# wukailu/single-stable-dreamfusion

Hardware: AMD Instinct MI355X
Metric: SDS train steps/sec + rays/sec at 128×128, 1/2/4/8 MI355X (higher is better)
Workload: dtype fp16+f32; 1 GPU; C2: -O (fp16, cuda_ray, dir_text) 128x128 render, batch 1, max_steps 512, density grid update every 16 steps; global_batch=1, parallelism=dp1, backward=fused, launch=hip-graph replay, grad_exchange=none (one rank), optimizer_in_graph=True

## Files before the change

### include/dfhip.h

```cpp
#ifndef DFHIP_H
#define DFHIP_H

#include <stdint.h>

#ifdef __cplusplus
extern "C" {
#endif

typedef void *dfhip_stream_t;

enum dfhip_dtype { DFHIP_F32 = 0, DFHIP_F16 = 1, DFHIP_F64 = 2, DFHIP_BF16 = 3 };
enum dfhip_shading {
    DFHIP_SHADING_ALBEDO = 0,
    DFHIP_SHADING_TEXTURELESS = 1,
    DFHIP_SHADING_LAMBERTIAN = 2,
    DFHIP_SHADING_NORMAL = 3
};

enum dfhip_status {
    DFHIP_OK = 0,
    DFHIP_EINVAL = 1,
    DFHIP_EDTYPE = 2,
    DFHIP_ELAUNCH = 3,
    DFHIP_ENOMEM = 4
// ... 444 lines not shown
                                              const int32_t *m_dev, uint32_t D, uint32_t C,
                                              uint32_t L, float S, uint32_t H, uint32_t gridtype,
                                              int align_corners, uint32_t group, float eps,
                                              uint32_t *entries, uint32_t *counts,
                                              float *partial, int accumulate,
                                              dfhip_stream_t stream);
typedef struct dfhip_binned_opts {
    int32_t walk_mode;
    int32_t fast_bin;
    int32_t walk_groups_per_cu;
    int32_t lane_perm;
    int32_t kept_clean;
    uint64_t *trace;
    float *found_inf;
    const uint32_t *row_live;
} dfhip_binned_opts;
int dfhip_grid_backward_binned_scratch_opts(uint32_t cap, const int32_t *offsets_host,
                                            uint32_t L, uint32_t C, uint32_t group,
                                            const dfhip_binned_opts *opts, uint64_t *entries_u32,
                                            uint64_t *counts_u32, uint64_t *partial_f32);
uint32_t dfhip_grid_backward_binned_tile(uint32_t group, const dfhip_binned_opts *opts);
int dfhip_grid_encode_backward_binned_opts(int phase, int grad_dtype, const void *grad_lbc,
                                           const float *inputs, float bound,
                                           const int32_t *offsets, const int32_t *offsets_host,
                                           float *grad_embeddings, uint32_t B,
                                           const int32_t *m_dev, uint32_t D, uint32_t C,
                                           uint32_t L, float S, uint32_t H, uint32_t gridtype,
                                           int align_corners, uint32_t group, float eps,
                                           uint32_t *entries, uint32_t *counts, float *partial,
                                           int accumulate, const dfhip_binned_opts *opts,
// ... 68 lines not shown
    const float *nears, const float *fars, const float *w1, const float *b1, const float *w2,
    const float *b2, float *out_image, float *out_depth, uint8_t *mask, const float *g_image,
    float *grad_image, float *grad_ws, float *partial, float *gw1, float *gb1, float *gw2,
    float *gb2, const float *grad_loss, float lambda, float *loss, float *found_inf,
    int defer_sum, dfhip_stream_t stream);

int dfhip_ray_chain_train(
    int rgb_dtype, const float *sigmas, const void *rgbs, const float *deltas,
    const int32_t *rays, uint32_t M, uint32_t N, float T_thresh, float *ws, float *depth,
    float *image, const float *rays_d, const float *nears, const float *fars, const float *w1,
    const float *b1, const float *w2, const float *b2, float *out_image, float *out_depth,
    uint8_t *mask, const float *g_image, float *grad_image, float *grad_ws, float *partial,
    float *gw1, float *gb1, float *gw2, float *gb2, const float *grad_loss, float lambda,
    float *loss, float *found_inf, int defer_sum, float *grad_sigmas, void *grad_rgbs,
    dfhip_stream_t stream);

int dfhip_entropy_forward(uint32_t N, const float *ws, float lambda, float *loss,
                          dfhip_stream_t stream);
int dfhip_entropy_backward(uint32_t N, const float *ws, const float *grad_loss, float lambda,
                           float *grad_ws, dfhip_stream_t stream);
int dfhip_entropy_backward_accumulate(uint32_t N, const float *ws, const float *grad_loss,
                                      float lambda, float *grad_ws, dfhip_stream_t stream);
int dfhip_opacity_forward(uint32_t N, const float *ws, float lambda, float *loss, int accumulate,
                          dfhip_stream_t stream);
int dfhip_opacity_backward_accumulate(uint32_t N, const float *ws, const float *grad_loss,
                                      float lambda, float *grad_ws, dfhip_stream_t stream);

int dfhip_train_step_prologue(const float *pose, float fx, float fy, float cx, float cy,
                              uint32_t H, uint32_t W, const float *aabb, float min_near,
                              uint64_t seed, uint64_t step, int perturb, const float *alphas,
// ... 141 lines not shown
```

### single-stable-dreamfusion_amd/_dfhip.py

```python
from __future__ import annotations

import ctypes
import os
from pathlib import Path

import torch

LIB_PATH = Path(os.environ.get("DFHIP_LIB", Path(__file__).resolve().parent / "lib" / "libdfhip.so"))

F32, F16, F64, BF16 = 0, 1, 2, 3
_DTYPE = {torch.float32: F32, torch.float16: F16, torch.float64: F64, torch.bfloat16: BF16}

_vp, _u32, _i32, _f32 = ctypes.c_void_p, ctypes.c_uint32, ctypes.c_int, ctypes.c_float
_u64 = ctypes.c_uint64

_SIGS = {
    "dfhip_near_far_from_aabb": [_i32, _vp, _vp, _vp, _u32, _f32, _vp, _vp, _vp],
    "dfhip_get_rays": [_vp, _f32, _f32, _f32, _f32, _u32, _u32, _vp, _vp, _vp],
    "dfhip_density_grid_ema": [_vp, _vp, _u32, _u32, _f32, _vp, _vp, _vp],
    "dfhip_packbits_mean": [_vp, _u32, _vp, _f32, _vp, _vp, _vp],
    "dfhip_mean_count": [_vp, _u32, _vp, _vp],
    "dfhip_sph_from_ray": [_i32, _vp, _vp, _f32, _u32, _vp, _vp],
    "dfhip_morton3D": [_vp, _u32, _vp, _vp],
    "dfhip_morton3D_invert": [_vp, _u32, _vp, _vp],
# ... 127 lines not shown
        _vp, _vp, _f32, _vp, _vp, _vp, _vp, _vp, _vp, _vp, _vp, _i32, _u32, _vp, _vp, _vp, _u32,
        _vp, _vp, _vp, _vp, _vp, _vp, _vp, _u32, _u32, _f32, _u32, _u32, _i32, _vp, _vp, _u32,
        _vp],
    "dfhip_adam_amp_step": [_i32, _vp, _vp, _vp, _vp, _vp, _vp, _vp, _vp, _vp, _vp, _vp, _vp,
                            _vp, _vp, _f32, _f32, _i32, _vp],
    "dfhip_adam_amp_step_lr_dev": [_i32, _vp, _vp, _vp, _vp, _vp, _vp, _vp, _vp, _vp, _vp, _vp,
                                   _vp, _vp, _vp, _vp, _f32, _f32, _i32, _vp],
    "dfhip_adam_amp_step_tail": [_i32, _vp, _vp, _vp, _vp, _vp, _vp, _vp, _vp, _vp, _vp, _vp,
                                 _vp, _vp, _vp, _vp, _f32, _f32, _i32, _u32, _vp, _vp, _vp, _vp],
    "dfhip_ray_head_backward_check": [_u32, _vp, _vp, _vp, _vp, _vp, _vp, _vp, _vp, _vp, _vp,
                                      _vp, _vp, _vp, _vp, _vp, _vp, _vp, _f32, _vp, _vp, _vp],
    "dfhip_ray_head_forward_backward_entropy_loss_check": [_u32] + [_vp] * 22 + [_f32, _vp, _vp,
                                                                                 _i32, _vp],
    "dfhip_ray_chain_train": [_i32] + [_vp] * 4 + [_u32, _u32, _f32] + [_vp] * 22 + [
        _f32, _vp, _vp, _i32, _vp, _vp, _vp],
    "dfhip_param_grad_sums": [_vp, _u32, _vp, _vp, _vp, _vp, _vp, _vp, _i32, _u32, _vp, _vp, _vp,
                              _vp, _vp, _vp, _f32, _vp, _vp, _vp],
    "dfhip_grid_field_backward_check": [_i32, _vp, _vp, _f32, _vp, _vp, _vp, _vp, _vp, _vp, _vp,
                                        _vp, _i32, _u32, _vp, _vp, _vp, _u32, _vp, _vp, _vp, _vp,
                                        _vp, _vp, _i32, _vp, _i32, _vp],
    "dfhip_grid_field_backward_check_live": [_i32, _vp, _vp, _f32, _vp, _vp, _vp, _vp, _vp, _vp,
                                             _vp, _vp, _i32, _u32, _vp, _vp, _vp, _u32, _vp, _vp,
                                             _vp, _vp, _vp, _vp, _i32, _vp, _i32, _vp, _vp],
    "dfhip_march_rays_train_count_staged_quads": [_i32, _vp, _vp, _vp, _f32, _f32, _u32, _u32,
                                                  _u32, _u32, _vp, _vp, _vp, _vp, _vp, _vp, _vp,
                                                  _i32, _vp, _vp, _u32, _f32, _u32, _u32, _i32,
                                                  _u32, _vp, _vp, _vp],
    "dfhip_train_step_prologue_row": [_vp, _f32, _f32, _f32, _f32, _u32, _u32, _vp, _f32,
                                      ctypes.c_uint64, ctypes.c_uint64, _i32, _vp, _u32, _u32,
                                      _vp, _vp, _vp, _vp, _vp, _vp, _vp, _vp, _vp, _u32, _vp,
# ... 249 lines not shown
```

### single-stable-dreamfusion_amd/_gridencoder.py

```python
import ctypes

import _dfhip as _d
from _dfhip import call, ptr, stream, checked


def _common(inputs, embeddings, offsets):
    checked(inputs, "inputs")
    if inputs.dtype.itemsize != 4 or not inputs.is_floating_point():
        raise RuntimeError("inputs must be a float32 tensor")
    checked(embeddings, "embeddings")
    checked(offsets, "offsets", "int")
    return _d.dtype_code(embeddings, "embeddings")


def grid_encode_forward(inputs, embeddings, offsets, outputs, B, D, C, L, S, H, dy_dx, gridtype,
                        align_corners):
    dt = _common(inputs, embeddings, offsets)
    checked(outputs, "outputs")
    call("dfhip_grid_encode_forward", dt, ptr(inputs), ptr(embeddings), ptr(offsets), ptr(outputs),
         B, D, C, L, S, H, ptr(dy_dx), gridtype, int(bool(align_corners)), stream())


def grid_encode_backward(grad, inputs, embeddings, offsets, grad_embeddings, B, D, C, L, S, H,
                         dy_dx, grad_inputs, gridtype, align_corners):
# ... 90 lines not shown
    checked(partial, "partial")
    if m_dev is not None:
        checked(m_dev, "m_dev", "int")
    call("dfhip_grid_encode_backward_sliced_dyn", _d.dtype_code(grad_lbc, "grad"),
         _d.dtype_code(grad_embeddings, "grad_embeddings"), ptr(grad_lbc), ptr(inputs),
         float(bound), ptr(offsets), ptr(grad_embeddings), total_rows, B, ptr(m_dev), D, C, L, S,
         H, gridtype, int(bool(align_corners)), ptr(partial), parts, int(bool(accumulate)),
         stream())



class BinnedOpts(ctypes.Structure):
    _fields_ = [("walk_mode", ctypes.c_int32), ("fast_bin", ctypes.c_int32),
                ("walk_groups_per_cu", ctypes.c_int32), ("lane_perm", ctypes.c_int32),
                ("kept_clean", ctypes.c_int32), ("trace", ctypes.c_void_p),
                ("found_inf", ctypes.c_void_p), ("row_live", ctypes.c_void_p)]

    def __init__(self, walk_mode=-1, fast_bin=-1, walk_groups_per_cu=0, lane_perm=-1,
                 trace=None, kept_clean=0, found_inf=None, row_live=None):
        super().__init__(int(walk_mode), int(fast_bin), int(walk_groups_per_cu), int(lane_perm),
                         int(kept_clean), None if trace is None else ptr(trace),
                         None if found_inf is None else ptr(found_inf),
                         None if row_live is None else ptr(row_live))


def _opts_ref(opts):
    return None if opts is None else ctypes.byref(opts)


def grid_backward_binned_tile(opts=None, group=1):
    return int(_d.load().dfhip_grid_backward_binned_tile(int(group), _opts_ref(opts)))


def grid_backward_binned_scratch(cap, offsets_host, L, C, opts=None, group=1):
    import numpy as np
    off = np.ascontiguousarray(offsets_host, dtype=np.int32)
    e, c, p = ctypes.c_uint64(), ctypes.c_uint64(), ctypes.c_uint64()
    call("dfhip_grid_backward_binned_scratch_opts", int(cap), off.ctypes.data, int(L), int(C),
# ... 43 lines not shown
```

### single-stable-dreamfusion_amd/csrc/gridbin.hip

```cpp
#include "grid_common.h"

#include <algorithm>

#include <type_traits>

namespace dfhip {
namespace gb {

using ge::Levels;
using ge::LevelCtx;
using ge::SliceDyn;
typedef unsigned long long u64;

constexpr uint32_t kTile = 1024;
constexpr uint32_t kMaxBins = 4096;
constexpr uint32_t kMaxSlices = 128;
constexpr uint32_t kSliceBytes = 128 * 1024;
constexpr uint32_t kTotSplit = 16;
constexpr uint32_t kIdBits = 10;
constexpr uint32_t kIdMask = (1u << kIdBits) - 1u;
static_assert(kTile == (1u << kIdBits), "ids fill the low kIdBits bits of an entry");
constexpr uint32_t kCentreCost = 4;
#ifndef DFHIP_SEG_COST
#define DFHIP_SEG_COST 48
// ... 17 lines not shown

__device__ __forceinline__ uint64_t trace_hw_id() {
    uint32_t xcc, hw;
    asm volatile("s_getreg_b32 %0, hwreg(HW_REG_XCC_ID)" : "=s"(xcc));
    asm volatile("s_getreg_b32 %0, hwreg(HW_REG_HW_ID)" : "=s"(hw));
    return ((uint64_t)xcc << 32) | hw;
}

#ifndef DFHIP_WALK_G_DEFAULT
#define DFHIP_WALK_G_DEFAULT 3
#endif
#ifndef DFHIP_WALK_MODE_DEFAULT
#define DFHIP_WALK_MODE_DEFAULT -1
#endif

struct Opts {
    int walk_mode;
    bool fast_bin;
    uint32_t walk_g;
    uint32_t lane_perm;
    bool clean;
    uint64_t *trace;
    float *found_inf;
    const uint32_t *row_live;
};

static bool resolve_opts(const dfhip_binned_opts *o, Opts &r) {
    r.walk_mode = DFHIP_WALK_MODE_DEFAULT;
    r.fast_bin = true;
    r.walk_g = DFHIP_WALK_G_DEFAULT;
    r.lane_perm = 1;
    r.clean = false;
    r.trace = nullptr;
    r.found_inf = nullptr;
    r.row_live = nullptr;
    if (!o) return true;
    if (o->walk_mode < -1 || o->walk_mode > 1) {
        set_error("binned backward: walk_mode must be -1, 0 or 1 (got %d)",
                  (int)o->walk_mode);
        return false;
    }
    if (o->walk_groups_per_cu < 0 || o->walk_groups_per_cu > 16) {
        set_error("binned backward: walk_groups_per_cu must be 0..16 (got %d)",
                  (int)o->walk_groups_per_cu);
        return false;
    }
    if (o->walk_mode >= 0) r.walk_mode = o->walk_mode;
    r.fast_bin = o->fast_bin != 0;
    if (o->walk_groups_per_cu > 0) r.walk_g = (uint32_t)o->walk_groups_per_cu;
    if (o->lane_perm >= 0) r.lane_perm = o->lane_perm != 0;
    r.clean = o->kept_clean > 0;
    r.trace = o->trace;
    r.found_inf = o->found_inf;
    r.row_live = o->row_live;
    return true;
}

static uint32_t slice_shift(uint32_t C) {
    uint32_t shift = 0;
    while ((2ull << shift) * 8ull * C <= kSliceBytes) ++shift;
    return shift;
}

static int flat_walk_mode(uint32_t group, const Opts &op);
static bool make_bins(const int32_t *offsets_host, uint32_t L, uint32_t C, uint32_t cap,
                      uint32_t group, const Opts &op, BinInfo &bi) {
    if (L == 0 || L > ge::kMaxLevels || C == 0) return false;
    bi.L = L;
    bi.trace = op.trace;
// ... 114 lines not shown
template <uint32_t W>
__device__ __forceinline__ void append(const uint64_t (&mask)[W], uint32_t b0, uint32_t *cnt,
                                       uint16_t *seg, uint16_t id, uint32_t tile) {
#pragma unroll
    for (uint32_t h = 0; h < W; ++h) {
        uint64_t mk = mask[h];
        while (mk) {
            const uint32_t b = b0 + (uint32_t)__builtin_ctzll(mk) + 64u * h;
            mk &= mk - 1;
            const uint32_t slot = atomicAdd(&cnt[b], 1u);
            seg[(size_t)b * tile + slot] = id;
        }
    }
}

__device__ __forceinline__ bool row_is_live(const uint32_t *__restrict__ live, uint32_t r) {
    return !live || ((live[r >> 5] >> (r & 31u)) & 1u) != 0u;
}

template <uint32_t W>
__device__ __forceinline__ void count_dead(const uint64_t (&mask)[W], uint32_t b0,
                                           uint32_t *dead) {
#pragma unroll
    for (uint32_t h = 0; h < W; ++h) {
        uint64_t mk = mask[h];
        while (mk) {
            atomicAdd(&dead[b0 + (uint32_t)__builtin_ctzll(mk) + 64u * h], 1u);
            mk &= mk - 1;
        }
    }
}

template <uint32_t D, bool POW2>
__global__ __launch_bounds__(1024) void k_bin(const float *__restrict__ inputs,
                                             const int32_t *__restrict__ offsets, Levels lv,
                                             BinInfo bi, uint32_t gridtype, int align_corners,
                                             SliceDyn dyn, float inv, uint32_t B,
                                             uint32_t *__restrict__ counts,
                                             uint16_t *__restrict__ entries,
                                             const uint32_t *__restrict__ row_live) {
    __shared__ uint32_t cnt[kMaxBins];
    __shared__ uint32_t dead[kMaxBins];
    const bool align = align_corners != 0;
    const uint32_t M = ge::dyn_count(dyn, B);
    const uint32_t T = bi.tile;
    const uint32_t ntiles = ceil_div(M, T);
    const uint32_t nb = bi.nbins;
    for (uint32_t tile = blockIdx.x; tile < ntiles; tile += gridDim.x) {
        for (uint32_t b = threadIdx.x; b < nb; b += blockDim.x) cnt[b] = dead[b] = 0;
        __syncthreads();
        uint16_t *seg = entries + (size_t)tile * nb * T;
        const uint32_t s_end = min(M, (tile + 1) * T);
        for (uint32_t s = tile * T + threadIdx.x; s < s_end; s += blockDim.x) {
            float x[D];
            const bool live = row_is_live(row_live, s);
// ... 122 lines not shown
                const uint32_t r = (bk >> 16) + __builtin_amdgcn_mbcnt_hi(
                                                    (uint32_t)(bs >> 32),
                                                    __builtin_amdgcn_mbcnt_lo((uint32_t)bs, 0u));
                sg[tile - 1u - r] = (uint16_t)(id | (m6 << kIdBits));
            }
        }
    }
}

template <bool POW2, uint32_t GROUP = 1>
__global__ __launch_bounds__(1024) void k_bin_fast(const float *__restrict__ inputs,
                                                  FastLevels fl, BinInfo bi, int align_corners,
                                                  SliceDyn dyn, float inv, uint32_t B,
                                                  uint32_t *__restrict__ counts,
                                                  uint16_t *__restrict__ entries,
                                                  const uint32_t *__restrict__ row_live,
                                                  Stencil st = Stencil{0.0f, 0.0f}) {
    __shared__ uint32_t cnt[kMaxBins];
    __shared__ uint32_t dead[GROUP == 1 ? kMaxBins : 1];
    const float half = align_corners ? 0.0f : 0.5f;
    const uint32_t M = ge::dyn_count(dyn, B);
    const uint32_t T = GROUP == 1 ? bi.tile : kTile;
    const uint32_t ntiles = ceil_div(M, T);
    const uint32_t nb = bi.nbins, shift = bi.shift, smask = (1u << bi.shift) - 1u;
    for (uint32_t tile = blockIdx.x; tile < ntiles; tile += gridDim.x) {
        for (uint32_t b = threadIdx.x; b < nb; b += blockDim.x) {
            cnt[b] = 0;
            if constexpr (GROUP == 1) dead[b] = 0;
        }
        __syncthreads();
        uint16_t *seg = entries + (size_t)tile * nb * T;
// ... 1167 lines not shown
        set_error("%s: null pointer", name);
        return DFHIP_EINVAL;
    }
    const ge::Levels lv = ge::make_levels(L, S, H);
    const ge::SliceDyn dyn{m_dev, bound};
    gb::FastLevels fl;
    const bool fast = gb::make_fast_levels(offsets_host, lv, bi, gridtype, align_corners != 0, fl);
    if (group != 1) {
        if (group != 7 || C != 2 || grad_dtype == DFHIP_F32 || !fast || !(bound > 0.0f) ||
            !(eps >= 0.0f)) {
            set_error("%s: stencil groups need group 7, C = 2, f16 / bf16 gradients, bound > 0, "
                      "eps >= 0 and a mask-form level layout", name);
            return DFHIP_EINVAL;
        }
    }
    if (group != 1 && op.row_live) {
        set_error("%s: row_live applies to single samples (group 1); stencil groups take no "
                  "mask", name);
        return DFHIP_EINVAL;
    }
    const gb::Stencil st{eps, bound};
    bi.clear_totals = 1u;
    if (phase & 1) {
        if (!op.clean || B == 0)
            (void)hipMemsetAsync(counts + bi.o_totals, 0,
                                 (size_t)(gb::counts_words(bi) - bi.o_totals) * sizeof(uint32_t),
                                 s);
        if (B > 0) {
            const uint32_t gbin = bi.tcap < 4096u ? bi.tcap : 4096u;
            const bool pow2 = ge::dyn_pow2(dyn.bound);
            const float inv = pow2 ? 1.0f / (2.0f * dyn.bound) : 0.0f;
// ... 121 lines not shown
```

### single-stable-dreamfusion_amd/csrc/head.hip

```cpp
#include "common.h"
#include "chain_common.h"
#include "field_common.h"

#include <math.h>

namespace dfhip {
namespace hd {

constexpr int kDeg = 6;
constexpr int kIn = 3 + 3 * 2 * kDeg;
constexpr int kHid = 64;
constexpr int kOut = 3;
constexpr int kW1 = kHid * kIn, kB1 = kHid, kW2 = kOut * kHid, kB2 = kOut;
constexpr int kParams = kW1 + kB1 + kW2 + kB2;
constexpr float kHalfPi = 3.141592653589793f / 2.0f;

__device__ __forceinline__ float r16(float x) { return (float)(half_t)f32_rounded(x); }

struct alignas(16) W {
    float w1t[kW1], b1[kB1], w2[kW2], b2[kB2];
};

__device__ __forceinline__ void load_w(W &w, const float *w1, const float *b1, const float *w2,
                                       const float *b2) {
// ... 280 lines not shown
    const void *rgbs;
    const float *deltas;
    const int32_t *rays;
    uint32_t M, N;
    float T_thresh;
    float *ws, *depth, *image;
    const float *rays_d, *nears, *fars, *w1, *b1, *w2, *b2;
    float *out_image, *out_depth;
    uint8_t *mask;
    const float *g_image;
    float *grad_image, *grad_ws, *partial;
    const float *ent_grad_loss;
    float ent_lambda;
    float *grad_sigmas;
    void *grad_rgbs;
};

template <typename rgb_t> struct RawWin {
    float sg = 0.0f, dt = 0.0f, dl = 0.0f;
    rgb_t c0 = (rgb_t)0.0f, c1 = (rgb_t)0.0f, c2 = (rgb_t)0.0f;
    bool in = false;
};

template <typename rgb_t>
__device__ __forceinline__ RawWin<rgb_t> load_win(const RayChainArgs &p, uint32_t offset,
                                                  uint32_t num, uint32_t base, int lane) {
    RawWin<rgb_t> v;
    v.in = base < num && (uint32_t)lane < num - base;
    if (v.in) {
        const size_t i = (size_t)offset + base + lane;
// ... 13 lines not shown
};
template <typename rgb_t> __device__ __forceinline__ WinOps win_ops(const RawWin<rgb_t> &v) {
    WinOps o;
    o.a = v.in ? 1.0f - __expf(-v.sg * v.dt) : 0.0f;
    o.om = 1.0f - o.a;
    o.cr = to_f(v.c0);
    o.cg = to_f(v.c1);
    o.cb = to_f(v.c2);
    return o;
}

#define DFHIP_16(STEP)                                                                      \
    STEP(0) STEP(1) STEP(2) STEP(3) STEP(4) STEP(5) STEP(6) STEP(7) STEP(8) STEP(9) STEP(10) \
    STEP(11) STEP(12) STEP(13) STEP(14) STEP(15)

template <typename rgb_t>
__global__ __launch_bounds__(kThreads) void k_ray_chain(RayChainArgs p) {
    __shared__ W w;
    __shared__ alignas(16) float s_x[kRays][kIn + 1];
    __shared__ half_t s_dh[kRays][kHid];
    __shared__ half_t s_h[kRays][kHid];
    __shared__ float s_do[kRays][4];
    const int q = threadIdx.x & (kSub - 1), r = threadIdx.x / kSub;
    const int row_shift = (int)(threadIdx.x & 48);
    const uint32_t N = p.N;
    const uint32_t n = blockIdx.x * kRays + r;
    const bool live = n < N;
    const float T_thresh = p.T_thresh;
    rgb_t *grad_rgbs = (rgb_t *)p.grad_rgbs;

    uint32_t offset = 0, num = 0, num_all = 0;
// ... 70 lines not shown
            const int j = kPer * q + jj;
            float a = 0.0f;
#pragma unroll
            for (int k = 0; k < kOut; ++k) a = fmaf(dout[k], w.w2[k * kHid + j], a);
            s_dh[r][j] = (half_t)(h[jj] > 0.0f ? r16(a) : 0.0f);
            s_h[r][j] = (half_t)h[jj];
        }
        if (q == 0)
#pragma unroll
            for (int k = 0; k < kOut; ++k) s_do[r][k] = dout[k];
    }

    const float gr = g[0], gg = g[1], gb = g[2];
#define DFHIP_SAMPLE_GRAD(I, WL, TL, RL, GL, BL, DT, CR, CG, CB)                              \
    {                                                                                         \
        grad_rgbs[3 * (I) + 0] = rm::grad_cast<float, rgb_t>(gr * (WL));                      \
        grad_rgbs[3 * (I) + 1] = rm::grad_cast<float, rgb_t>(gg * (WL));                      \
        grad_rgbs[3 * (I) + 2] = rm::grad_cast<float, rgb_t>(gb * (WL));                      \
        float acc = fmaf(gr, fmaf((TL), (CR), -(rf - (RL))), gg * fmaf((TL), (CG), -(gf - (GL)))); \
        acc = fmaf(gb, fmaf((TL), (CB), -(bf - (BL))), acc);                                  \
        acc = fmaf(gw, 1.0f - wsv, acc);                                                      \
        p.grad_sigmas[(I)] = (DT) * acc;                                                      \
    }
    uint32_t done = 0;
    rm::BwdChain b;
    for (uint32_t base = 0; base < num && b.alive; base += 16) {
        cur = load_win<rgb_t>(p, offset, num, base, q);
        const WinOps v = win_ops(cur);
        b.wl = b.Tl = b.rl = b.gl = b.bl = 0.0f;
        b.taken = false;
#define DFHIP_BSTEP(J) b.step<J>(q, v.a, v.om, v.cr, v.cg, v.cb, T_thresh);
        DFHIP_16(DFHIP_BSTEP)
#undef DFHIP_BSTEP
        const bool taken = b.taken && cur.in;
        if (taken) {
            const size_t i = (size_t)offset + base + q;
            DFHIP_SAMPLE_GRAD(i, b.wl, b.Tl, b.rl, b.gl, b.bl, cur.dt, v.cr, v.cg, v.cb)
        }
        done = base + (uint32_t)__popcll((__ballot(taken) >> row_shift) & 0xFFFFull);
    }
#undef DFHIP_SAMPLE_GRAD
    if (live) {
        const uint64_t end = min((uint64_t)offset + num_all, (uint64_t)p.M);
        for (uint64_t row = (uint64_t)offset + done + q; row < end; row += 16) {
            p.grad_sigmas[row] = 0.0f;
            grad_rgbs[3 * row] = (rgb_t)0.0f;
            grad_rgbs[3 * row + 1] = (rgb_t)0.0f;
            grad_rgbs[3 * row + 2] = (rgb_t)0.0f;
        }
    }
    __syncthreads();
    write_partials(s_x, s_dh, s_h, s_do, p.partial);
}
#undef DFHIP_16

__device__ __forceinline__ void entropy_loss_block(uint32_t N, const float *__restrict__ ws,
                                                   float lambda, float *__restrict__ loss);

__device__ __forceinline__ void wsum_block(uint32_t blk, const float *__restrict__ partial,
                                           uint32_t blocks, float *gw1, float *gb1, float *gw2,
                                           float *gb2, float *found_inf) {
    __shared__ float red[16][64];
    const int o = threadIdx.x & 63, grp = threadIdx.x >> 6;
// ... 334 lines not shown
    if (N == 0) {
        set_error("%s: N must be > 0", name);
        return DFHIP_EINVAL;
    }
    if (!w1 || !depth || !image || !nears || !fars || !out_image || !out_depth || !mask ||
        !grad_loss) {
        set_error("%s: null pointer (the combined launch needs the background network)", name);
        return DFHIP_EINVAL;
    }
    const hd::FwdIO io{depth, image, nears, fars, out_image, out_depth, mask};
    return ray_head_backward(N, g_image, ws, rays_d, w1, b1, w2, b2, nullptr, grad_image,
                             grad_ws, nullptr, partial, gw1, gb1, gw2, gb2, grad_loss, lambda,
                             stream, loss, &io, found_inf, defer_sum != 0);
}

extern "C" int dfhip_ray_chain_train(
    int rgb_dtype, const float *sigmas, const void *rgbs, const float *deltas,
    const int32_t *rays, uint32_t M, uint32_t N, float T_thresh, float *ws, float *depth,
    float *image, const float *rays_d, const float *nears, const float *fars, const float *w1,
    const float *b1, const float *w2, const float *b2, float *out_image, float *out_depth,
    uint8_t *mask, const float *g_image, float *grad_image, float *grad_ws, float *partial,
    float *gw1, float *gb1, float *gw2, float *gb2, const float *grad_loss, float lambda,
    float *loss, float *found_inf, int defer_sum, float *grad_sigmas, void *grad_rgbs,
    dfhip_stream_t stream) {
    const char *name = "ray_chain_train";
    if (N == 0) {
        set_error("%s: N must be > 0", name);
        return DFHIP_EINVAL;
    }
    if (!sigmas || !rgbs || !deltas || !rays || !ws || !depth || !image || !rays_d || !nears ||
        !fars || !w1 || !b1 || !w2 || !b2 || !out_image || !out_depth || !mask || !g_image ||
        !grad_image || !grad_ws || !partial || !gw1 || !gb1 || !gw2 || !gb2 || !grad_loss ||
        !loss || !grad_sigmas || !grad_rgbs) {
        set_error("%s: null pointer (only found_inf may be null)", name);
        return DFHIP_EINVAL;
    }
    const hd::RayChainArgs a{sigmas, rgbs, deltas, rays, M, N, T_thresh, ws, depth, image,
                             rays_d, nears, fars, w1, b1, w2, b2, out_image, out_depth, mask,
                             g_image, grad_image, grad_ws, partial, grad_loss, lambda,
                             grad_sigmas, grad_rgbs};
    hipStream_t s = as_stream(stream);
    const uint32_t blocks = ceil_div(N, (uint32_t)hd::kRays);
    if (rgb_dtype == DFHIP_F32) hd::k_ray_chain<float><<<blocks, hd::kThreads, 0, s>>>(a);
    else if (rgb_dtype == DFHIP_F16) hd::k_ray_chain<half_t><<<blocks, hd::kThreads, 0, s>>>(a);
    else if (rgb_dtype == DFHIP_BF16) hd::k_ray_chain<bf16_t><<<blocks, hd::kThreads, 0, s>>>(a);
    else {
        set_error("%s: rgb dtype must be f32, f16 or bf16 (got %d)", name, rgb_dtype);
        return DFHIP_EDTYPE;
    }
    if (!defer_sum)
        hd::k_head_wsum<<<ceil_div((uint32_t)hd::kParams, 64u) + 1u, 1024, 0, s>>>(
            partial, blocks, gw1, gb1, gw2, gb2, ws, N, lambda, loss, found_inf);
    return check_launch(name);
}

extern "C" int dfhip_param_grad_sums(const float *mlp_partial, uint32_t mlp_parts, float *gw1,
                                     float *gb1, float *gw2, float *gb2, float *gw3, float *gb3,
                                     int accumulate, uint32_t N, const float *head_partial,
                                     float *hgw1, float *hgb1, float *hgw2, float *hgb2,
                                     const float *ws, float lambda, float *loss,
                                     float *found_inf, dfhip_stream_t stream) {
    const char *name = "param_grad_sums";
    if (!mlp_partial || mlp_parts == 0 || !gw1 || !gb1 || !gw2 || !gb2 || !gw3 || !gb3) {
        set_error("%s: null pointer or no parts in the field role", name);
        return DFHIP_EINVAL;
    }
    if (head_partial && (N == 0 || !hgw1 || !hgb1 || !hgw2 || !hgb2)) {
        set_error("%s: the head role needs N > 0 and its four gradients", name);
// ... 74 lines not shown
```

### single-stable-dreamfusion_amd/nerf/native_step.py

```python
import ctypes

import numpy as np
import torch

import _dfhip
import _fieldmlp
import _gridencoder
import _raymarching
from _dfhip import call, ptr, stream


SHADINGS = {"albedo": 0, "textureless": 1, "lambertian": 2}
FD_EPS = 1e-2


def eligible(trainer, shading):
    from .sd import InjectedSDS
    m, opt = trainer.model, trainer.opt
    if shading not in SHADINGS or not isinstance(trainer.guidance, InjectedSDS):
        return False
    if shading != "albedo" and not trainer.fused_backward:
        return False
    if not ((trainer.fp16 or getattr(trainer, "bf16", False)) and m.cuda_ray):
        return False
# ... 102 lines not shown
        self.grad_sigma = torch.empty(cap, **f32)
        self.grad_albedo = torch.empty(fcap, 3, **f16)
        self.grad_sigma_field = (torch.empty(fcap, **f32) if self.shade_code
                                 else self.grad_sigma)
        self.d_enc = torch.empty(self.L, fcap, self.C, **f16)
        self.mlp_partial = torch.empty(_fieldmlp.backward_parts(fcap) * _fieldmlp.params_count(),
                                       **f32)
        self.stencil_bin = bool(self.shade_code) and bool(getattr(trainer, "stencil_bin", True))
        ne, nc, npf = _gridencoder.grid_backward_binned_scratch(
            cap if self.stencil_bin else fcap, enc.offsets_host, self.L, self.C,
            group=7 if self.stencil_bin else 1)
        self.bin_scratch = (torch.empty(ne, **i32), torch.zeros(nc, **i32),
                            torch.empty(npf, **f32))
        self.live_mask = (bool(getattr(trainer, "live_mask", True)) and trainer.fused_backward
                          and not self.stencil_bin)
        self.row_live = torch.zeros((fcap + 31) // 32, **i32)
        sc = trainer.scaler
        if sc.is_enabled() and sc._scale is None:
            sc._lazy_init_scale_growth_tracker(dev)
        self._ones = torch.ones(1, **f32)
        from .utils import flat_grad_bucket_
        self.grad_bucket = flat_grad_bucket_(m.parameters())
        self.two_pass = not trainer.fused_backward
        if self.two_pass:
            self.d_enc2 = torch.empty_like(self.d_enc)
            self.zero_image = torch.zeros(N, 3, **f32)
            self.grad_ws2 = torch.empty(N, **f32)
            self.grad_sigma2 = torch.empty(cap, **f32)
            self.grad_albedo2 = torch.empty(cap, 3, **f16)
            self._emb_launch2 = None
        self.params = [p for p in m.parameters() if p.requires_grad]
# ... 111 lines not shown
        rgb = self.albedo
        if self.shade_code:
            with T("shading_forward", 0, md, 28 + 3 * hb + 12 + 4 + 3 * hb + 12):
                call(self._shade_fwd, ptr(self.sigma_field), ptr(self.albedo),
                     ptr(self.dirs), ptr(self.light), self.ratio, FD_EPS, self.shade_code,
                     ptr(self.m_dev), cap, ptr(self.sigma), ptr(self.color), ptr(self.normal),
                     ptr(self.orient_partial), self.lam_orient, ptr(self.orient), None, stream())
            rgb = self.color
        bw = self._bg_weights()
        combined = (not self.two_pass and self.lam > 0 and bw[0] is not None
                    and bool(getattr(self.trainer, "combined_head", True)))
        fi = self.found_inf
        defer = combined and self.merged_sums
        chain = defer and bool(getattr(self.trainer, "fused_ray_chain", True))
        self.ray_chain = chain
        if chain:
            with T("ray_chain", (32 + 120 + 44) * N, md,
                   (4 + 3 * hb + 8) + (4 + 3 * hb + 8 + 4 + 3 * hb)):
                call("dfhip_ray_chain_train", _dfhip._DTYPE[rgb.dtype], ptr(self.sigma), ptr(rgb),
                     ptr(self.deltas), ptr(self.rays), cap, N, 1e-4, ptr(self.ws),
                     ptr(self.depth), ptr(self.image), ptr(self.rays_d), ptr(self.nears),
                     ptr(self.fars), *[ptr(w) for w in bw], ptr(self.out_image),
                     ptr(self.out_depth), ptr(self.mask), ptr(self.g_image),
                     ptr(self.grad_image), ptr(self.grad_ws), ptr(self.head_partial),
                     *[ptr(g) for g in self._bg_grads()], ptr(scale), self.lam, ptr(self.loss),
                     ptr(fi), 1, ptr(self.grad_sigma), ptr(self.grad_albedo), stream())
            return self._field_backward(fi, defer, hb)
        with T("composite_rays_train_forward", 32 * N, md, 4 + 3 * hb + 8):
            _raymarching.composite_rays_train_forward_mixed(
                self.sigma, rgb, self.deltas, self.rays, cap, N, 1e-4, self.ws, self.depth,
                self.image)
        if not combined:
            with T("ray_head_forward", 60 * N):
                call("dfhip_ray_head_forward", N, ptr(self.ws), ptr(self.depth), ptr(self.image),
                     ptr(self.rays_d), ptr(self.nears), ptr(self.fars), *[ptr(w) for w in bw],
                     ptr(self.bg_color), ptr(self.out_image), ptr(self.out_depth),
                     ptr(self.mask), stream())
        if self.two_pass:
            if self.lam > 0:
                call("dfhip_entropy_forward", N, ptr(self.ws), self.lam, ptr(self.loss),
                     stream())
# ... 44 lines not shown
        return self._field_backward(fi, defer, hb)

    def _field_backward(self, fi, defer, hb):
        from gridencoder.grid import _parts
        m, N, T, mf = self.trainer.model, self.N, _dfhip.timed, self.m_field
        S, Hb, gridtype, align, _ = self.meta
        gbw = self._bg_grads()
        per_bwd = 2 * self.L * self.C * hb + 4 + 3 * hb + 12
        with T("field_mlp_backward", 4 * _fieldmlp.params_count(), mf, per_bwd):
            _fieldmlp.grid_field_backward(
                self.enc, self.xyz_field, m.bound, self.mlp, self.grad_sigma_field,
                self.grad_albedo, self.d_enc, self.mlp_partial, [p.grad for p in self.mlp],
                self.encoder.offsets, self.rows, S, Hb, gridtype, align, None, None,
                _parts(self.rows, self.C), self.m_field, found_inf=fi,
                defer_sum=self.merged_sums,
                row_live=self.row_live if self.live_mask else None)
            if self.merged_sums:
                call("dfhip_param_grad_sums", ptr(self.mlp_partial),
                     _fieldmlp.backward_parts(self.fcap) if self.fcap else 1,
                     *[ptr(p.grad) for p in self.mlp], 0, N,
                     ptr(self.head_partial) if defer else None,
                     *[ptr(g) if defer else None for g in gbw],
                     ptr(self.ws) if defer else None, self.lam,
                     ptr(self.loss) if defer else None, ptr(fi), stream())
        return self.loss

    def _backward_two_pass(self, bw, scale):
        m = self.trainer.model
        N, cap = self.N, self.cap
        S, Hb, gridtype, align, _ = self.meta
        from gridencoder.grid import _parts
# ... 60 lines not shown
            args = (self.d_enc, self.xyz_field, m.bound, self.encoder.offsets, offsets_host,
                    self.encoder.embeddings.grad, self.fcap, self.m_field, 3, self.C, self.L, S,
                    Hb, gridtype, align, *self.bin_scratch)
            kw = {}
        kw["opts"] = self._kept_clean_opts()
        self._emb_launch = _gridencoder.binned_launcher(*args, **kw)

    def clear_found_inf(self):
        if self.found_inf is not None:
            self.found_inf.zero_()

    def _kept_clean_opts(self):
        o = self.binned_opts if self.binned_opts is not None else _gridencoder.BinnedOpts()
        o.kept_clean = 1 if getattr(self.trainer, "kept_clean_scratch", True) else 0
        o.found_inf = ptr(self.found_inf)
        o.row_live = ptr(self.row_live) if self.live_mask else None
        return o

    def time_field(self, reps=5):
        m = self.trainer.model
        S, Hb, gridtype, align, _ = self.meta
        from gridencoder.grid import _parts

        def fwd():
            _fieldmlp.grid_field_forward(self.xyz_field, m.bound, self.table,
                                         self.encoder.offsets, S, Hb, gridtype, align, self.mlp,
                                         self.enc, self.sigma_field, self.albedo, self.m_field,
                                         quads=self.quads)

        def bwd():
            _fieldmlp.grid_field_backward(
                self.enc, self.xyz_field, m.bound, self.mlp, self.grad_sigma_field,
# ... 39 lines not shown
```

### single-stable-dreamfusion_amd/nerf/utils.py

```python
import glob
import math
import os
import random
import time

import numpy as np
import torch
import torch.distributed as dist
import torch.nn as nn
import torch.nn.functional as F


def custom_meshgrid(*args):
    return torch.meshgrid(*args, indexing="ij")


def safe_normalize(x, eps=1e-20):
    return x / torch.sqrt(torch.clamp(torch.sum(x * x, -1, keepdim=True), min=eps))


@torch.autocast("cuda", enabled=False)
def get_rays(poses, intrinsics, H, W, N=-1, error_map=None):
    device = poses.device
    B = poses.shape[0]
# ... 208 lines not shown
        self.fused_backward = fused_backward
        self.graph_step = graph_step
        self.dp_in_graph = None
        self._graphs = {}
        self.native_optimizer = True
        self.native_step = True
        self.stencil_bin = True
        self.kept_clean_scratch = True
        self.live_mask = True
        self.combined_head = True
        self.fold_overflow_check = True
        self.merged_grad_sums = True
        self.store_live_count = True
        self.quads_in_march = True
        self.fused_ray_chain = True
        self.module_buckets = True
        self.native_losses = True
        self._native_opt = None
        self.step_hook = None
        self.device = device if device is not None else torch.device(
            f"cuda:{local_rank}" if torch.cuda.is_available() else "cpu")

        model.to(self.device)
        self.model = model
        if world_size > 1 and dist.is_available() and dist.is_initialized():
            with torch.no_grad():
                for t in list(model.parameters()) + list(model.buffers()):
                    dist.broadcast(t.data, src=0)
        self._capture_stream = None
        if (self.device.type == "cuda" and dist.is_available() and dist.is_initialized()
# ... 436 lines not shown
```

Baseline: 20.79 million rays/s.

## Emit per-sample live byte mask from fused ray chain for grid backward

The fused ray-chain kernel now writes a per-sample byte flag marking rows whose sigma or rgb gradient is nonzero. The binned grid-encoder backward reads this byte mask in place of the bit mask that the field backward previously produced. This is meant to drop the separate bit-mask generation and let the grid backward skip dead rows straight from the chain's output. It adds a byte store per sample in the chain kernel. It also adds a slow host-side property that rebuilds the bit mask for debugging.

```diff
diff --git a/include/dfhip.h b/include/dfhip.h
--- a/include/dfhip.h
+++ b/include/dfhip.h
@@ -482,6 +482,7 @@
     uint64_t *trace;
     float *found_inf;
     const uint32_t *row_live;
+    const uint8_t *row_live_bytes;
 } dfhip_binned_opts;
 int dfhip_grid_backward_binned_scratch_opts(uint32_t cap, const int32_t *offsets_host,
                                             uint32_t L, uint32_t C, uint32_t group,
@@ -580,6 +581,15 @@
     float *gw1, float *gb1, float *gw2, float *gb2, const float *grad_loss, float lambda,
     float *loss, float *found_inf, int defer_sum, float *grad_sigmas, void *grad_rgbs,
     dfhip_stream_t stream);
+int dfhip_ray_chain_train_live(
+    int rgb_dtype, const float *sigmas, const void *rgbs, const float *deltas,
+    const int32_t *rays, uint32_t M, uint32_t N, float T_thresh, float *ws, float *depth,
+    float *image, const float *rays_d, const float *nears, const float *fars, const float *w1,
+    const float *b1, const float *w2, const float *b2, float *out_image, float *out_depth,
+    uint8_t *mask, const float *g_image, float *grad_image, float *grad_ws, float *partial,
+    float *gw1, float *gb1, float *gw2, float *gb2, const float *grad_loss, float lambda,
+    float *loss, float *found_inf, int defer_sum, float *grad_sigmas, void *grad_rgbs,
+    uint8_t *row_live_bytes, dfhip_stream_t stream);
 
 int dfhip_entropy_forward(uint32_t N, const float *ws, float lambda, float *loss,
                           dfhip_stream_t stream);
diff --git a/single-stable-dreamfusion_amd/_dfhip.py b/single-stable-dreamfusion_amd/_dfhip.py
--- a/single-stable-dreamfusion_amd/_dfhip.py
+++ b/single-stable-dreamfusion_amd/_dfhip.py
@@ -165,6 +165,8 @@
                                                                                  _i32, _vp],
     "dfhip_ray_chain_train": [_i32] + [_vp] * 4 + [_u32, _u32, _f32] + [_vp] * 22 + [
         _f32, _vp, _vp, _i32, _vp, _vp, _vp],
+    "dfhip_ray_chain_train_live": [_i32] + [_vp] * 4 + [_u32, _u32, _f32] + [_vp] * 22 + [
+        _f32, _vp, _vp, _i32, _vp, _vp, _vp, _vp],
     "dfhip_param_grad_sums": [_vp, _u32, _vp, _vp, _vp, _vp, _vp, _vp, _i32, _u32, _vp, _vp, _vp,
                               _vp, _vp, _vp, _f32, _vp, _vp, _vp],
     "dfhip_grid_field_backward_check": [_i32, _vp, _vp, _f32, _vp, _vp, _vp, _vp, _vp, _vp, _vp,
diff --git a/single-stable-dreamfusion_amd/_gridencoder.py b/single-stable-dreamfusion_amd/_gridencoder.py
--- a/single-stable-dreamfusion_amd/_gridencoder.py
+++ b/single-stable-dreamfusion_amd/_gridencoder.py
@@ -128,14 +128,16 @@
     _fields_ = [("walk_mode", ctypes.c_int32), ("fast_bin", ctypes.c_int32),
                 ("walk_groups_per_cu", ctypes.c_int32), ("lane_perm", ctypes.c_int32),
                 ("kept_clean", ctypes.c_int32), ("trace", ctypes.c_void_p),
-                ("found_inf", ctypes.c_void_p), ("row_live", ctypes.c_void_p)]
+                ("found_inf", ctypes.c_void_p), ("row_live", ctypes.c_void_p),
+                ("row_live_bytes", ctypes.c_void_p)]
 
     def __init__(self, walk_mode=-1, fast_bin=-1, walk_groups_per_cu=0, lane_perm=-1,
-                 trace=None, kept_clean=0, found_inf=None, row_live=None):
+                 trace=None, kept_clean=0, found_inf=None, row_live=None, row_live_bytes=None):
         super().__init__(int(walk_mode), int(fast_bin), int(walk_groups_per_cu), int(lane_perm),
                          int(kept_clean), None if trace is None else ptr(trace),
                          None if found_inf is None else ptr(found_inf),
-                         None if row_live is None else ptr(row_live))
+                         None if row_live is None else ptr(row_live),
+                         None if row_live_bytes is None else ptr(row_live_bytes))
 
 
 def _opts_ref(opts):
diff --git a/single-stable-dreamfusion_amd/csrc/gridbin.hip b/single-stable-dreamfusion_amd/csrc/gridbin.hip
--- a/single-stable-dreamfusion_amd/csrc/gridbin.hip
+++ b/single-stable-dreamfusion_amd/csrc/gridbin.hip
@@ -55,6 +55,11 @@
 #define DFHIP_WALK_MODE_DEFAULT -1
 #endif
 
+struct RowLive {
+    const uint32_t *bits;
+    const uint8_t *bytes;
+};
+
 struct Opts {
     int walk_mode;
     bool fast_bin;
@@ -63,7 +68,7 @@
     bool clean;
     uint64_t *trace;
     float *found_inf;
-    const uint32_t *row_live;
+    RowLive row_live;
 };
 
 static bool resolve_opts(const dfhip_binned_opts *o, Opts &r) {
@@ -74,8 +79,12 @@
     r.clean = false;
     r.trace = nullptr;
     r.found_inf = nullptr;
-    r.row_live = nullptr;
+    r.row_live = RowLive{nullptr, nullptr};
     if (!o) return true;
+    if (o->row_live && o->row_live_bytes) {
+        set_error("binned backward: row_live and row_live_bytes are exclusive");
+        return false;
+    }
     if (o->walk_mode < -1 || o->walk_mode > 1) {
         set_error("binned backward: walk_mode must be -1, 0 or 1 (got %d)",
                   (int)o->walk_mode);
@@ -93,7 +102,7 @@
     r.clean = o->kept_clean > 0;
     r.trace = o->trace;
     r.found_inf = o->found_inf;
-    r.row_live = o->row_live;
+    r.row_live = RowLive{o->row_live, o->row_live_bytes};
     return true;
 }
 
@@ -238,8 +247,9 @@
     }
 }
 
-__device__ __forceinline__ bool row_is_live(const uint32_t *__restrict__ live, uint32_t r) {
-    return !live || ((live[r >> 5] >> (r & 31u)) & 1u) != 0u;
+__device__ __forceinline__ bool row_is_live(const RowLive &live, uint32_t r) {
+    if (live.bytes) return live.bytes[r] != 0;
+    return !live.bits || ((live.bits[r >> 5] >> (r & 31u)) & 1u) != 0u;
 }
 
 template <uint32_t W>
@@ -262,7 +272,7 @@
                                              SliceDyn dyn, float inv, uint32_t B,
                                              uint32_t *__restrict__ counts,
                                              uint16_t *__restrict__ entries,
-                                             const uint32_t *__restrict__ row_live) {
+                                             RowLive row_live) {
     __shared__ uint32_t cnt[kMaxBins];
     __shared__ uint32_t dead[kMaxBins];
     const bool align = align_corners != 0;
@@ -415,7 +425,7 @@
                                                   SliceDyn dyn, float inv, uint32_t B,
                                                   uint32_t *__restrict__ counts,
                                                   uint16_t *__restrict__ entries,
-                                                  const uint32_t *__restrict__ row_live,
+                                                  RowLive row_live,
                                                   Stencil st = Stencil{0.0f, 0.0f}) {
     __shared__ uint32_t cnt[kMaxBins];
     __shared__ uint32_t dead[GROUP == 1 ? kMaxBins : 1];
@@ -1613,7 +1623,7 @@
             return DFHIP_EINVAL;
         }
     }
-    if (group != 1 && op.row_live) {
+    if (group != 1 && (op.row_live.bits || op.row_live.bytes)) {
         set_error("%s: row_live applies to single samples (group 1); stencil groups take no "
                   "mask", name);
         return DFHIP_EINVAL;
diff --git a/single-stable-dreamfusion_amd/csrc/head.hip b/single-stable-dreamfusion_amd/csrc/head.hip
--- a/single-stable-dreamfusion_amd/csrc/head.hip
+++ b/single-stable-dreamfusion_amd/csrc/head.hip
@@ -318,6 +318,7 @@
     float ent_lambda;
     float *grad_sigmas;
     void *grad_rgbs;
+    uint8_t *row_live;
 };
 
 template <typename rgb_t> struct RawWin {
@@ -361,7 +362,7 @@
     STEP(0) STEP(1) STEP(2) STEP(3) STEP(4) STEP(5) STEP(6) STEP(7) STEP(8) STEP(9) STEP(10) \
     STEP(11) STEP(12) STEP(13) STEP(14) STEP(15)
 
-template <typename rgb_t>
+template <typename rgb_t, bool LIVE = false>
 __global__ __launch_bounds__(kThreads) void k_ray_chain(RayChainArgs p) {
     __shared__ W w;
     __shared__ alignas(16) float s_x[kRays][kIn + 1];
@@ -462,13 +463,22 @@
     const float gr = g[0], gg = g[1], gb = g[2];
 #define DFHIP_SAMPLE_GRAD(I, WL, TL, RL, GL, BL, DT, CR, CG, CB)                              \
     {                                                                                         \
-        grad_rgbs[3 * (I) + 0] = rm::grad_cast<float, rgb_t>(gr * (WL));                      \
-        grad_rgbs[3 * (I) + 1] = rm::grad_cast<float, rgb_t>(gg * (WL));                      \
-        grad_rgbs[3 * (I) + 2] = rm::grad_cast<float, rgb_t>(gb * (WL));                      \
+        const rgb_t c0 = rm::grad_cast<float, rgb_t>(gr * (WL));                              \
+        const rgb_t c1 = rm::grad_cast<float, rgb_t>(gg * (WL));                              \
+        const rgb_t c2 = rm::grad_cast<float, rgb_t>(gb * (WL));                              \
+        grad_rgbs[3 * (I) + 0] = c0;                                                          \
+        grad_rgbs[3 * (I) + 1] = c1;                                                          \
+        grad_rgbs[3 * (I) + 2] = c2;                                                          \
         float acc = fmaf(gr, fmaf((TL), (CR), -(rf - (RL))), gg * fmaf((TL), (CG), -(gf - (GL)))); \
         acc = fmaf(gb, fmaf((TL), (CB), -(bf - (BL))), acc);                                  \
         acc = fmaf(gw, 1.0f - wsv, acc);                                                      \
-        p.grad_sigmas[(I)] = (DT) * acc;                                                      \
+        const float gs = (DT) * acc;                                                          \
+        p.grad_sigmas[(I)] = gs;                                                              \
+                     \
+                     \
+        if constexpr (LIVE)                                                                   \
+            p.row_live[(I)] = (gs != 0.0f || to_f(c0) != 0.0f || to_f(c1) != 0.0f ||          \
+                               to_f(c2) != 0.0f) ? 1 : 0;                                     \
     }
     uint32_t done = 0;
     rm::BwdChain b;
@@ -495,6 +505,7 @@
             grad_rgbs[3 * row] = (rgb_t)0.0f;
             grad_rgbs[3 * row + 1] = (rgb_t)0.0f;
             grad_rgbs[3 * row + 2] = (rgb_t)0.0f;
+            if constexpr (LIVE) p.row_live[row] = 0;
         }
     }
     __syncthreads();
@@ -859,6 +870,49 @@
                              stream, loss, &io, found_inf, defer_sum != 0);
 }
 
+static int ray_chain_train(
+    const char *name, int rgb_dtype, const float *sigmas, const void *rgbs, const float *deltas,
+    const int32_t *rays, uint32_t M, uint32_t N, float T_thresh, float *ws, float *depth,
+    float *image, const float *rays_d, const float *nears, const float *fars, const float *w1,
+    const float *b1, const float *w2, const float *b2, float *out_image, float *out_depth,
+    uint8_t *mask, const float *g_image, float *grad_image, float *grad_ws, float *partial,
+    float *gw1, float *gb1, float *gw2, float *gb2, const float *grad_loss, float lambda,
+    float *loss, float *found_inf, int defer_sum, float *grad_sigmas, void *grad_rgbs,
+    uint8_t *row_live, dfhip_stream_t stream) {
+    if (N == 0) {
+        set_error("%s: N must be > 0", name);
+        return DFHIP_EINVAL;
+    }
+    if (!sigmas || !rgbs || !deltas || !rays || !ws || !depth || !image || !rays_d || !nears ||
+        !fars || !w1 || !b1 || !w2 || !b2 || !out_image || !out_depth || !mask || !g_image ||
+        !grad_image || !grad_ws || !partial || !gw1 || !gb1 || !gw2 || !gb2 || !grad_loss ||
+        !loss || !grad_sigmas || !grad_rgbs) {
+        set_error("%s: null pointer (only found_inf may be null)", name);
+        return DFHIP_EINVAL;
+    }
+    const hd::RayChainArgs a{sigmas, rgbs, deltas, rays, M, N, T_thresh, ws, depth, image,
+                             rays_d, nears, fars, w1, b1, w2, b2, out_image, out_depth, mask,
+                             g_image, grad_image, grad_ws, partial, grad_loss, lambda,
+                             grad_sigmas, grad_rgbs, row_live};
+    hipStream_t s = as_stream(stream);
+    const uint32_t blocks = ceil_div(N, (uint32_t)hd::kRays);
+#define DFHIP_RAY_CHAIN(T)                                                            \
+    (row_live ? hd::k_ray_chain<T, true> : hd::k_ray_chain<T, false>)                 \
+        <<<blocks, hd::kThreads, 0, s>>>(a)
+    if (rgb_dtype == DFHIP_F32) DFHIP_RAY_CHAIN(float);
+    else if (rgb_dtype == DFHIP_F16) DFHIP_RAY_CHAIN(half_t);
+    else if (rgb_dtype == DFHIP_BF16) DFHIP_RAY_CHAIN(bf16_t);
+    else {
+        set_error("%s: rgb dtype must be f32, f16 or bf16 (got %d)", name, rgb_dtype);
+        return DFHIP_EDTYPE;
+    }
+    if (!defer_sum)
+        hd::k_head_wsum<<<ceil_div((uint32_t)hd::kParams, 64u) + 1u, 1024, 0, s>>>(
+            partial, blocks, gw1, gb1, gw2, gb2, ws, N, lambda, loss, found_inf);
+    return check_launch(name);
+}
+#undef DFHIP_RAY_CHAIN
+
 extern "C" int dfhip_ray_chain_train(
     int rgb_dtype, const float *sigmas, const void *rgbs, const float *deltas,
     const int32_t *rays, uint32_t M, uint32_t N, float T_thresh, float *ws, float *depth,
@@ -868,35 +922,31 @@
     float *gw1, float *gb1, float *gw2, float *gb2, const float *grad_loss, float lambda,
     float *loss, float *found_inf, int defer_sum, float *grad_sigmas, void *grad_rgbs,
     dfhip_stream_t stream) {
-    const char *name = "ray_chain_train";
-    if (N == 0) {
-        set_error("%s: N must be > 0", name);
-        return DFHIP_EINVAL;
-    }
-    if (!sigmas || !rgbs || !deltas || !rays || !ws || !depth || !image || !rays_d || !nears ||
-        !fars || !w1 || !b1 || !w2 || !b2 || !out_image || !out_depth || !mask || !g_image ||
-        !grad_image || !grad_ws || !partial || !gw1 || !gb1 || !gw2 || !gb2 || !grad_loss ||
-        !loss || !grad_sigmas || !grad_rgbs) {
-        set_error("%s: null pointer (only found_inf may be null)", name);
-        return DFHIP_EINVAL;
-    }
-    const hd::RayChainArgs a{sigmas, rgbs, deltas, rays, M, N, T_thresh, ws, depth, image,
-                             rays_d, nears, fars, w1, b1, w2, b2, out_image, out_depth, mask,
-                             g_image, grad_image, grad_ws, partial, grad_loss, lambda,
-                             grad_sigmas, grad_rgbs};
-    hipStream_t s = as_stream(stream);
-    const uint32_t blocks = ceil_div(N, (uint32_t)hd::kRays);
-    if (rgb_dtype == DFHIP_F32) hd::k_ray_chain<float><<<blocks, hd::kThreads, 0, s>>>(a);
-    else if (rgb_dtype == DFHIP_F16) hd::k_ray_chain<half_t><<<blocks, hd::kThreads, 0, s>>>(a);
-    else if (rgb_dtype == DFHIP_BF16) hd::k_ray_chain<bf16_t><<<blocks, hd::kThreads, 0, s>>>(a);
-    else {
-        set_error("%s: rgb dtype must be f32, f16 or bf16 (got %d)", name, rgb_dtype);
-        return DFHIP_EDTYPE;
-    }
-    if (!defer_sum)
-        hd::k_head_wsum<<<ceil_div((uint32_t)hd::kParams, 64u) + 1u, 1024, 0, s>>>(
-            partial, blocks, gw1, gb1, gw2, gb2, ws, N, lambda, loss, found_inf);
-    return check_launch(name);
+    return ray_chain_train("ray_chain_train", rgb_dtype, sigmas, rgbs, deltas, rays, M, N,
+                           T_thresh, ws, depth, image, rays_d, nears, fars, w1, b1, w2, b2,
+                           out_image, out_depth, mask, g_image, grad_image, grad_ws, partial, gw1,
+                           gb1, gw2, gb2, grad_loss, lambda, loss, found_inf, defer_sum,
+                           grad_sigmas, grad_rgbs, nullptr, stream);
+}
+
+extern "C" int dfhip_ray_chain_train_live(
+    int rgb_dtype, const float *sigmas, const void *rgbs, const float *deltas,
+    const int32_t *rays, uint32_t M, uint32_t N, float T_thresh, float *ws, float *depth,
+    float *image, const float *rays_d, const float *nears, const float *fars, const float *w1,
+    const float *b1, const float *w2, const float *b2, float *out_image, float *out_depth,
+    uint8_t *mask, const float *g_image, float *grad_image, float *grad_ws, float *partial,
+    float *gw1, float *gb1, float *gw2, float *gb2, const float *grad_loss, float lambda,
+    float *loss, float *found_inf, int defer_sum, float *grad_sigmas, void *grad_rgbs,
+    uint8_t *row_live_bytes, dfhip_stream_t stream) {
+    if (!row_live_bytes) {
+        set_error("ray_chain_train_live: null row_live_bytes");
+        return DFHIP_EINVAL;
+    }
+    return ray_chain_train("ray_chain_train_live", rgb_dtype, sigmas, rgbs, deltas, rays, M, N,
+                           T_thresh, ws, depth, image, rays_d, nears, fars, w1, b1, w2, b2,
+                           out_image, out_depth, mask, g_image, grad_image, grad_ws, partial, gw1,
+                           gb1, gw2, gb2, grad_loss, lambda, loss, found_inf, defer_sum,
+                           grad_sigmas, grad_rgbs, row_live_bytes, stream);
 }
 
 extern "C" int dfhip_param_grad_sums(const float *mlp_partial, uint32_t mlp_parts, float *gw1,
diff --git a/single-stable-dreamfusion_amd/nerf/native_step.py b/single-stable-dreamfusion_amd/nerf/native_step.py
--- a/single-stable-dreamfusion_amd/nerf/native_step.py
+++ b/single-stable-dreamfusion_amd/nerf/native_step.py
@@ -140,7 +140,11 @@
                             torch.empty(npf, **f32))
         self.live_mask = (bool(getattr(trainer, "live_mask", True)) and trainer.fused_backward
                           and not self.stencil_bin)
-        self.row_live = torch.zeros((fcap + 31) // 32, **i32)
+        self._row_live_bits = torch.zeros((fcap + 31) // 32, **i32)
+        self.chain_live = False
+        self._launcher_chain_live = False
+        self.row_live_bytes = (torch.zeros(cap, dtype=torch.uint8, device=dev)
+                               if self.live_mask and not self.shade_code else None)
         sc = trainer.scaler
         if sc.is_enabled() and sc._scale is None:
             sc._lazy_init_scale_growth_tracker(dev)
@@ -282,17 +286,23 @@
         defer = combined and self.merged_sums
         chain = defer and bool(getattr(self.trainer, "fused_ray_chain", True))
         self.ray_chain = chain
+        self.chain_live = (chain and self.live_mask and self.row_live_bytes is not None
+                           and bool(getattr(self.trainer, "chain_live_mask", True)))
+        if self._emb_launch is not None and self.chain_live != self._launcher_chain_live:
+            self._emb_launch = self._emb_launch2 = None
         if chain:
+            live = (ptr(self.row_live_bytes),) if self.chain_live else ()
             with T("ray_chain", (32 + 120 + 44) * N, md,
-                   (4 + 3 * hb + 8) + (4 + 3 * hb + 8 + 4 + 3 * hb)):
-                call("dfhip_ray_chain_train", _dfhip._DTYPE[rgb.dtype], ptr(self.sigma), ptr(rgb),
+                   (4 + 3 * hb + 8) + (4 + 3 * hb + 8 + 4 + 3 * hb) + len(live)):
+                call("dfhip_ray_chain_train" + ("_live" if live else ""),
+                     _dfhip._DTYPE[rgb.dtype], ptr(self.sigma), ptr(rgb),
                      ptr(self.deltas), ptr(self.rays), cap, N, 1e-4, ptr(self.ws),
                      ptr(self.depth), ptr(self.image), ptr(self.rays_d), ptr(self.nears),
                      ptr(self.fars), *[ptr(w) for w in bw], ptr(self.out_image),
                      ptr(self.out_depth), ptr(self.mask), ptr(self.g_image),
                      ptr(self.grad_image), ptr(self.grad_ws), ptr(self.head_partial),
                      *[ptr(g) for g in self._bg_grads()], ptr(scale), self.lam, ptr(self.loss),
-                     ptr(fi), 1, ptr(self.grad_sigma), ptr(self.grad_albedo), stream())
+                     ptr(fi), 1, ptr(self.grad_sigma), ptr(self.grad_albedo), *live, stream())
             return self._field_backward(fi, defer, hb)
         with T("composite_rays_train_forward", 32 * N, md, 4 + 3 * hb + 8):
             _raymarching.composite_rays_train_forward_mixed(
@@ -367,7 +377,8 @@
                 self.encoder.offsets, self.rows, S, Hb, gridtype, align, None, None,
                 _parts(self.rows, self.C), self.m_field, found_inf=fi,
                 defer_sum=self.merged_sums,
-                row_live=self.row_live if self.live_mask else None)
+                row_live=(self._row_live_bits if self.live_mask and not self.chain_live
+                          else None))
             if self.merged_sums:
                 call("dfhip_param_grad_sums", ptr(self.mlp_partial),
                      _fieldmlp.backward_parts(self.fcap) if self.fcap else 1,
@@ -458,8 +469,22 @@
         o = self.binned_opts if self.binned_opts is not None else _gridencoder.BinnedOpts()
         o.kept_clean = 1 if getattr(self.trainer, "kept_clean_scratch", True) else 0
         o.found_inf = ptr(self.found_inf)
-        o.row_live = ptr(self.row_live) if self.live_mask else None
+        bits = self.live_mask and not self.chain_live
+        o.row_live = ptr(self._row_live_bits) if bits else None
+        o.row_live_bytes = ptr(self.row_live_bytes) if self.chain_live else None
+        self._launcher_chain_live = self.chain_live
         return o
+
+    @property
+    def row_live(self):
+        if not self.chain_live:
+            return self._row_live_bits
+        m = int(self.m_field[0])
+        bits = torch.zeros(self._row_live_bits.numel() * 32, dtype=torch.int64,
+                           device=self.row_live_bytes.device)
+        bits[:m] = self.row_live_bytes[:m] != 0
+        words = (bits.view(-1, 32) << torch.arange(32, device=bits.device)).sum(1)
+        return words.to(torch.int32)
 
     def time_field(self, reps=5):
         m = self.trainer.model
diff --git a/single-stable-dreamfusion_amd/nerf/utils.py b/single-stable-dreamfusion_amd/nerf/utils.py
--- a/single-stable-dreamfusion_amd/nerf/utils.py
+++ b/single-stable-dreamfusion_amd/nerf/utils.py
@@ -246,6 +246,7 @@
         self.store_live_count = True
         self.quads_in_march = True
         self.fused_ray_chain = True
+        self.chain_live_mask = True
         self.module_buckets = True
         self.native_losses = True
         self._native_opt = None
```

Result: faster. 21.18 million rays/s, median of 6 (+1.9%).
